# Mikata-Project/adcraft

Hardware: AMD Instinct MI355X
Metric: env-steps/sec (envs×keywords auctions/s) (higher is better)
Workload: dtype i32 cents + f32 (Philox4x32-7 u32); 1 GPU; cfg2: 4096 envs x 256 keywords per GPU, IMPLICIT keywords, mean_volume 128, cvr 0.8, no_vol_prob 0.0, drift False, budget non-binding, 60-step episodes with auto-reset; envs_per_gpu=4096, keywords=256, parallelism=env-sharded x1, collective=none (single GPU), weak_scaling_reference=also.cfg4.value of the N=1 --full line (same per-GPU shard as the N>1 runs)

## Files before the change

adcraft_amd/_ffi.py:

```python
import ctypes as C
import os

from . import build as _build

ADC_OK, ADC_EINVAL, ADC_EHIP, ADC_ENOMEM, ADC_ESTATE, ADC_ETYPE, ADC_ERCCL = 0, -1, -2, -3, -4, -5, -6
MODEL_IMPLICIT, MODEL_EXPLICIT, MODEL_IMPLICIT_GENERAL = 0, 1, 2
P_VOL_MEAN, P_VOL_STD, P_A, P_B, P_BCTR, P_SCTR, P_REV_MEAN, P_REV_STD, P_COUNT = range(9)
(BUF_PARAMS, BUF_BIDS, BUF_BUDGET, BUF_IMPRESSIONS, BUF_CLICKS, BUF_CONVERSIONS, BUF_COST, BUF_REVENUE, BUF_REWARD,
 BUF_CUM_PROFIT, BUF_DAYS, BUF_TERMINATED, BUF_TRUNCATED, BUF_METRIC_PROFIT, BUF_METRIC_SCALARS, BUF_FLAT_OBS,
 BUF_ROLLOUT_ACTION, BUF_ROLLOUT_LOGP, BUF_ROLLOUT_VALUE, BUF_ROLLOUT_REWARD, BUF_ROLLOUT_TERMINATED, BUF_ROLLOUT_TRUNCATED,
 BUF_ROLLOUT_OBS) = range(23)
MLP_TANH, MLP_RELU = 0, 1
ES_CENTERED_RANK, ES_RAW = 0, 1
ES_ADAM, ES_SGD = 0, 1
ROLLOUT_OBS = 1


class EngineError(RuntimeError):
    pass


class EngineStateError(AssertionError):
    """ADC_ESTATE: the call is not valid in the engine's current state (step before reset, a step whose clicks can no longer be
    replayed ...).  An AssertionError, as the reference raises for step-before-reset (gymnasium_kw_env.py:194-196), but one of its
# ... 128 lines not shown
        "adc_engine_stream": ([vp, C.POINTER(vp)], C.c_int),
        "adc_engine_sample_actions": ([vp, f32, f32, f32], C.c_int),
        "adc_engine_set_flat_actions_device": ([vp, vp], C.c_int),
        "adc_engine_flat_obs_enable": ([vp, C.c_int], C.c_int),
        "adc_engine_profile_enable": ([vp, C.c_int], C.c_int),
        "adc_engine_profile_sample_every": ([vp, C.c_int32], C.c_int),
        "adc_engine_profile_read": ([vp, vp, C.POINTER(i64)], C.c_int),
        "adc_engine_profile_records": ([vp, C.POINTER(i64)], C.c_int),
        "adc_engine_region_begin": ([vp], C.c_int),
        "adc_engine_region_end": ([vp, C.POINTER(f64)], C.c_int),
        "adc_engine_comm_stats": ([vp, C.POINTER(i64), C.POINTER(f64), C.POINTER(f64), C.c_int], C.c_int),
        "adc_engine_step_kernel_name": ([vp], C.c_char_p),
        "adc_engine_metrics_enable": ([vp, C.c_int], C.c_int),
        "adc_engine_metrics_reset": ([vp], C.c_int),
        "adc_engine_metrics_read": ([vp, vp, vp], C.c_int),
        "adc_engine_ideal_profit": ([vp, C.c_int, vp, C.c_int, vp], C.c_int),
        "adc_bid_curves_from_samples": ([C.c_int, vp, i32, vp, i32, vp, vp], C.c_int),
        "adc_engine_metrics_akncp_ncp": ([vp, f64, vp, vp], C.c_int),
        "adc_engine_bid_curves_contenders": ([vp, vp, vp, C.POINTER(i32)], C.c_int),
        "adc_engine_outcomes_replay": ([vp, i32, i32, vp, f32, i64, vp, vp, vp, vp, C.POINTER(i64), vp], C.c_int),
        "adc_engine_outcomes_replay_tape": ([vp, i32, vp, f32, C.POINTER(Tape), i64, vp, vp, vp, vp, C.POINTER(i64), vp], C.c_int),
        "adc_nth_price_auction": ([C.c_int, f64, vp, i32, i32, i32, i32, C.POINTER(i32), vp, vp], C.c_int),
        "adc_sigmoid": ([f64, f64, f64], f64),
        "adc_clamp": ([f64, f64, f64], f64),
        "adc_threshold_sigmoid": ([f64, f64, f64, f64], f64),
        "adc_sum_f64": ([vp, i64], f64),
        "adc_count_true": ([vp, i64], i64),
        "adc_nonneg_int_normal": ([f64, f64, u64, u64], u64),
        "adc_binomial": ([u64, f64, u64, u64], u64),
        "adc_cost_create": ([f64, i64, u64, u64, vp], C.c_int),
        "adc_auction_word_intervals": ([f32, f32, f32, f32, vp], C.c_int),
        "adc_auction_word_brackets": ([f32, f32, f32, f32, vp], C.c_int),
        "adc_check_win_brackets": ([i64, vp, vp, vp, vp, vp, vp, vp], i64),
        "adc_sample_random_keyword": ([C.c_uint64, C.c_uint32, C.c_uint32, vp], C.c_int),
        "adc_interp_act_host": ([f32, i32, f32, i32, C.c_double, C.c_double, C.c_double, vp, i32, i32, vp, vp, i32, vp, vp,
                                 C.c_double, vp, vp, vp, vp, vp], C.c_int),
        "adc_interp_key_host": ([f32], C.c_double),
        "adc_engine_mlp_init": ([vp, C.POINTER(MLPConfig), vp], C.c_int),
        "adc_engine_mlp_set_layer": ([vp, i32, i32, vp, vp], C.c_int),
        "adc_engine_mlp_set_norm": ([vp, vp, vp], C.c_int),
        "adc_engine_mlp_set_log_std": ([vp, vp], C.c_int),
        "adc_engine_mlp_set_deterministic": ([vp, i32], C.c_int),
        "adc_engine_mlp_act": ([vp, f32, vp], C.c_int),
        "adc_engine_mlp_step": ([vp, f32], C.c_int),
        "adc_engine_mlp_last": ([vp, vp, vp, vp, vp, vp], C.c_int),
        "adc_engine_mlp_bootstrap_value": ([vp, vp], C.c_int),
        "adc_engine_rollout_enable": ([vp, i32, i32], C.c_int),
        "adc_engine_rollout_reset": ([vp], C.c_int),
        "adc_engine_rollout_fetch": ([vp, C.POINTER(i32), vp, vp, vp, vp, vp, vp, vp], C.c_int),
        "adc_engine_mlp_population": ([vp, i32, vp], C.c_int),
        "adc_engine_mlp_set_member_layer": ([vp, i32, i32, vp, vp], C.c_int),
        "adc_engine_mlp_param_count": ([vp, C.POINTER(i64)], C.c_int),
        "adc_engine_mlp_get_params": ([vp, vp], C.c_int),
        "adc_engine_mlp_get_member_params": ([vp, i32, vp], C.c_int),
        "adc_engine_es_init": ([vp, C.POINTER(ESConfig)], C.c_int),
        "adc_engine_es_perturb": ([vp], C.c_int),
        "adc_engine_es_fitness": ([vp, vp], C.c_int),
        "adc_engine_es_update": ([vp, vp, C.POINTER(ESStats)], C.c_int),
        "adc_engine_es_state_get": ([vp, vp, vp, vp, C.POINTER(i64)], C.c_int),
        "adc_engine_es_state_set": ([vp, vp, vp, vp, i64], C.c_int),
        "adc_es_config_check": ([C.POINTER(ESConfig), C.POINTER(C.c_char_p)], C.c_int),
        "adc_es_noise_host": ([u64, C.c_uint32, C.c_uint32, i64, i64, vp], C.c_int),
        "adc_es_update_host": ([C.POINTER(ESConfig), u64, i32, i64, vp, i64, vp, vp, vp, vp], C.c_int),
        "adc_mlp_config_check": ([C.POINTER(MLPConfig), i32, C.POINTER(C.c_char_p)], C.c_int),
        "adc_mlp_act_host": ([C.POINTER(MLPConfig), i32, vp, vp, vp, vp, vp, vp, vp, vp, vp, u64, C.c_uint32, f32,
                              vp, vp, vp, vp, vp, vp, vp], C.c_int),
        "adc_mlp_math_host": ([i32, f32], f32),
        "adc_mlp_math_sweep_host": ([i32, f32, f32, vp, vp], i64),
        "adc_mlp_agent_key_host": ([u64], u64),
        "adc_mlp_default_agent_key_host": ([u64, u64], u64),
        "adc_explicit_curve_host": ([C.c_uint64, C.c_uint32, i32, i32, f32, f32, f32, vp, i32, vp, vp, vp], C.c_int),
        "adc_debug_win_brackets_device": ([C.c_int, i64, vp, vp, vp, vp, vp], C.c_int),
        "adc_debug_philox_device": ([C.c_int, i64, vp, vp, vp], C.c_int),
        "adc_debug_walk_stats": ([vp, vp, C.c_int], C.c_int),
        "adc_debug_direct_days": ([vp, vp, C.c_int], C.c_int),
        "adc_debug_chain_device": ([C.c_int, f64, i64, vp, vp], C.c_int),
        "adc_engine_env_groups": ([vp, vp], C.c_int),
        "adc_engine_set_env_groups": ([vp, C.c_int32], C.c_int),
        "adc_comm_get_unique_id": ([vp], C.c_int),
        "adc_engine_comm_init": ([vp, vp, i32, i32], C.c_int),
        "adc_engine_comm_destroy": ([vp], C.c_int),
        "adc_engine_comm_info": ([vp, vp, vp], C.c_int),
        "adc_engine_metrics_allreduce": ([vp, vp, vp, vp], C.c_int),
        "adc_engine_comm_allreduce_f64": ([vp, vp, i32, i32], C.c_int),
    }
    for name, (args, res) in sig.items():
        fn = getattr(L, name)
        fn.argtypes = args
        fn.restype = res
    if L.adc_abi_version() != ABI_VERSION or L.adc_stream_revision() != STREAM_REVISION:
        raise EngineError(f"{path}: ABI version {L.adc_abi_version()} / stream revision {L.adc_stream_revision()}, this package "
                          f"expects {ABI_VERSION} / {STREAM_REVISION} (a stale build?)")
    _lib = L
    return L


EXPORTED = None


def check(rc):
    if rc == ADC_OK:
        return
    msg = (lib().adc_last_error() or b"").decode("utf-8", "replace")
    if rc == ADC_EINVAL:
        raise ValueError(msg)
# ... 18 lines not shown
```

adcraft_amd/csrc/adc_law.h:

```cpp
#pragma once
#include <stdint.h>

#if defined(__HIPCC__)
#include <hip/hip_runtime.h>
#define ADC_HD __host__ __device__ __forceinline__
#else
#include <math.h>
#define ADC_HD static inline
#endif

namespace adc {

enum Stage : uint32_t { ST_VOL = 0, ST_AUCTION = 1, ST_DRIFT = 2, ST_XPHANTOM = 3, ST_XREV = 4, ST_ACTION = 5, ST_METRIC = 6, ST_CONV = 7, ST_KEYGEN = 8, ST_AGENT = 9,
                        ST_GBIDDERS = 10, ST_GBID = 11, ST_GCLICK = 12, ST_INTERP = 13, ST_MLP = 14 };
constexpr int kTimesteps = 24;
constexpr int kVolumeMax = 1 << 20;
constexpr float kMoneyMaxCents = 1.0e9f;

struct U4 { uint32_t x, y, z, w; };

ADC_HD uint32_t xor3(uint32_t a, uint32_t b, uint32_t c)
{
#if defined(__HIP_DEVICE_COMPILE__)
    return __builtin_amdgcn_bitop3_b32(a, b, c, 0x96);
// ... 331 lines not shown
ADC_HD int32_t competitor_cents_from_v(uint32_t v24, float loc, float scale, Tab tab)
{
    const float x = fma32(__builtin_fabsf(scale), laplace_deviate_from_v(v24, tab), loc);
    float c = __builtin_rintf(__builtin_fabsf(x) * 100.0f);
    c = c < kMoneyMaxCents ? c : kMoneyMaxCents;
    return (int32_t)c;
}

ADC_HD uint32_t auction_uniform24(uint32_t w, const AuctionLaw &a, bool &click)
{
    click = bernoulli32(w, a.t32);
    const uint32_t d = click ? w : w - a.t32;
    const uint32_t v = mulhi32(d, click ? a.m_click : a.m_noclick);
    return v < 0x00FFFFFFu ? v : 0x00FFFFFFu;
}

ADC_HD bool auction_wins(uint32_t w, int32_t bid_c, int32_t comp_c) { return bid_c > comp_c && w != 0xFFFFFFFFu; }

template <typename Tab>
ADC_HD int32_t auction_outcome_unless_top_word(uint32_t w, const AuctionLaw &a, float loc, float scale, Tab tab, bool &click)
{
    click = w < a.t32;
    const uint32_t d = click ? w : w - a.t32;
    const uint32_t v = mulhi32(d, click ? a.m_click : a.m_noclick);
    return competitor_cents_from_v(v < 0x00FFFFFFu ? v : 0x00FFFFFFu, loc, scale, tab);
}

ADC_HD int32_t auction_outcome(uint32_t w, const AuctionLaw &a, float loc, float scale, const LogTableEntry *tab, bool &click)
{
    return competitor_cents_from_v(auction_uniform24(w, a, click), loc, scale, tab);
}


ADC_HD uint32_t lower_bound_v(int32_t target, float loc, float scale, const LogTableEntry *tab)
{
    const float s = __builtin_fabsf(scale);
    const float x_t = ((float)target - 0.5f) * 0.01f;
    const float z_t = (x_t - loc) / s;
    const float e_t = __builtin_fabsf(z_t);
#if defined(__HIP_DEVICE_COMPILE__)
    float mag_f = __builtin_amdgcn_exp2f(fma32(e_t, -1.44269504f, 23.0f));
#else
    float mag_f = exp2f(fma32(e_t, -1.44269504f, 23.0f));
#endif
    mag_f = mag_f < 8388607.0f ? mag_f : 8388607.0f;
    mag_f = mag_f > 0.0f ? mag_f : 0.0f;
    const uint32_t mag = (uint32_t)mag_f;
    const uint32_t est = z_t < 0.0f ? mag : 0x00FFFFFFu - mag;
    float slack = mag_f * (6.0e-6f + 2.4e-7f * (__builtin_fabsf(x_t) + __builtin_fabsf(loc)) / s);
    slack = slack < 4194304.0f ? slack : 4194304.0f;
    const uint32_t half = 8u + (uint32_t)slack;
    uint32_t lo = est > half ? est - half : 0u;
    uint32_t hi = est + half < 0x01000000u ? est + half : 0x01000000u;
    if (lo > 0u && !(signed_cents_from_v(lo - 1u, loc, scale, tab) < target)) lo = 0u;
    if (hi < 0x01000000u && !(signed_cents_from_v(hi, loc, scale, tab) >= target)) hi = 0x01000000u;
    while (lo < hi) {
        const uint32_t mid = (lo + hi) >> 1;
        if (signed_cents_from_v(mid, loc, scale, tab) >= target) hi = mid;
        else lo = mid + 1u;
    }
    return lo;
}

ADC_HD uint64_t offset_reaching(uint32_t W, uint32_t m, uint64_t range)
{
    if (W == 0u) return 0ull;
    if (W > 0x00FFFFFFu || m == 0u) return range;
    const double q = ((double)W * 4294967296.0) / (double)m;
    if (!(q < (double)range)) return range;
    uint64_t d = (uint64_t)q;
    const uint64_t need = (uint64_t)W << 32;
    if (d * m >= need) { if (d > 0ull && (d - 1ull) * m >= need) d -= 1ull; }
    else { d += 1ull; if (d * m < need) d += 1ull; }
    return d < range ? d : range;
}

struct WinIntervals { uint32_t c_lo, c_w, n_lo, n_w; };

ADC_HD WinIntervals win_intervals(int32_t bid_c, float loc, float scale, uint64_t t_click, const AuctionLaw &law, const LogTableEntry *tab)
{
    const uint32_t w_lo = lower_bound_v(1 - bid_c, loc, scale, tab);
    const uint32_t w_hi = lower_bound_v(bid_c, loc, scale, tab);
    WinIntervals r{0u, 0u, 0u, 0u};
    if (!(w_lo < w_hi)) return r;
    const uint64_t top = 0xFFFFFFFFull;
    uint64_t a = offset_reaching(w_lo, law.m_click, t_click), b = offset_reaching(w_hi, law.m_click, t_click);
    b = b < top ? b : top;
    if (a < b) { r.c_lo = (uint32_t)a; r.c_w = (uint32_t)(b - a); }
    const uint64_t range_n = 4294967296ull - t_click;
    a = t_click + offset_reaching(w_lo, law.m_noclick, range_n);
    b = t_click + offset_reaching(w_hi, law.m_noclick, range_n);
    b = b < top ? b : top;
    if (a < b) { r.n_lo = (uint32_t)a; r.n_w = (uint32_t)(b - a); }
    return r;
}

struct WinBrackets { WinIntervals out, in; };
constexpr float kWordSlack = 4096.0f;

ADC_HD float fast_exp2(float x)
{
#if defined(__HIP_DEVICE_COMPILE__)
    return __builtin_amdgcn_exp2f(x);
#else
    return exp2f(x);
#endif
}
ADC_HD float fast_rcp(float x)
{
#if defined(__HIP_DEVICE_COMPILE__)
    return __builtin_amdgcn_rcpf(x);
#else
    return 1.0f / x;
#endif
}
ADC_HD float min_num(float a, float b) { return __builtin_fminf(a, b); }
ADC_HD float max_num(float a, float b) { return __builtin_fmaxf(a, b); }
ADC_HD uint32_t sat_sub(uint32_t a, uint32_t b)
{
#if defined(__clang__)
    return __builtin_elementwise_sub_sat(a, b);
#else
    return a > b ? a - b : 0u;
#endif
}
ADC_HD uint32_t to_word(float x)
{
#if defined(__HIP_DEVICE_COMPILE__)
    return (uint32_t)x;
#else
    return !(x > 0.0f) ? 0u : x >= 4294967296.0f ? 0xFFFFFFFFu : (uint32_t)x;
#endif
}

ADC_HD void lower_bound_estimate(float x_t, float loc, float inv_s, float &est, float &slack)
{
    const float z_t = (x_t - loc) * inv_s;
    const float e_t = __builtin_fabsf(z_t);
    const float mag = min_num(fast_exp2(fma32(e_t, -1.44269504f, 23.0f)), 8388607.0f);
    est = z_t < 0.0f ? mag : 16777215.0f - mag;
    const float rel = fma32(1.0e-6f, fma32(__builtin_fabsf(x_t) + __builtin_fabsf(loc), inv_s, e_t), 2.0e-5f);
    slack = min_num(fma32(mag, rel, 16.0f), 33554432.0f);
}

ADC_HD WinBrackets win_brackets(int32_t bid_c, float loc, float scale, float t_f)
{
    const float inv_s = fast_rcp(__builtin_fabsf(scale));
    const float bc = (float)bid_c;
    float lo, lo_s, hi, hi_s;
    lower_bound_estimate(fma32(bc, -0.01f, 0.005f), loc, inv_s, lo, lo_s);
    lower_bound_estimate(fma32(bc, 0.01f, -0.005f), loc, inv_s, hi, hi_s);
    const float lo_out = lo - lo_s, lo_in = lo + lo_s, hi_out = hi + hi_s, hi_in = hi - hi_s;
    const float a_c = max_num(t_f * 5.9604644775390625e-08f, 1.0f);
    const float a_n = max_num((4294967296.0f - t_f) * 5.9604644775390625e-08f, 1.0f);
    const float t_dn = t_f - kWordSlack, t_up = t_f + kWordSlack;
    WinBrackets r;
    const uint32_t c_lo_out = to_word(fma32(lo_out, a_c, -kWordSlack)), c_hi_out = to_word(min_num(fma32(hi_out, a_c, kWordSlack), t_f));
    const uint32_t c_lo_in = to_word(fma32(lo_in, a_c, kWordSlack)), c_hi_in = to_word(min_num(fma32(hi_in, a_c, -kWordSlack), t_f));
    const uint32_t n_lo_out = to_word(fma32(lo_out, a_n, t_dn)), n_hi_out = to_word(fma32(hi_out, a_n, t_up));
    const uint32_t n_lo_in = to_word(fma32(lo_in, a_n, t_up)), n_hi_in = to_word(fma32(hi_in, a_n, t_dn));
    r.out = WinIntervals{c_lo_out, sat_sub(c_hi_out, c_lo_out), n_lo_out, sat_sub(n_hi_out, n_lo_out)};
    r.in = WinIntervals{c_lo_in, sat_sub(c_hi_in, c_lo_in), n_lo_in, sat_sub(n_hi_in, n_lo_in)};
    return r;
}

ADC_HD void clicked_win_interval(int32_t bid_c, float loc, float scale, uint64_t t_click, const AuctionLaw &law, const LogTableEntry *tab,
                                 uint32_t &lo, uint32_t &width)
{
    lo = 0u;
    width = 0u;
    const uint32_t w_lo = lower_bound_v(1 - bid_c, loc, scale, tab), w_hi = lower_bound_v(bid_c, loc, scale, tab);
    if (!(w_lo < w_hi)) return;
    const uint64_t a = offset_reaching(w_lo, law.m_click, t_click);
    uint64_t b = offset_reaching(w_hi, law.m_click, t_click);
    b = b < 0xFFFFFFFFull ? b : 0xFFFFFFFFull;
    if (a < b) { lo = (uint32_t)a; width = (uint32_t)(b - a); }
}

ADC_HD int32_t revenue_cents_tab(uint32_t w, float mu, float sd, const NormTableEntry *tab)
{
    float x = fma32(sd, normal_tab(w, tab), mu);
    x = x > 0.01f ? x : 0.01f;
    return money_to_cents(x);
}

ADC_HD int32_t revenue_cents(uint32_t w, float mu, float sd)
{
    float x = fma32(sd, normal_from_word(w), mu);
    x = x > 0.01f ? x : 0.01f;
    return money_to_cents(x);
}

ADC_HD int32_t volume_from_word(uint32_t w, float mean, float sd, const NormTableEntry *tab)
{
    float x = fma32(sd, normal_tab(w, tab), mean);
    x = x > 0.0f ? x : 0.0f;
    x = x < (float)kVolumeMax ? x : (float)kVolumeMax;
    const float t = __builtin_truncf(x);
    return (int32_t)t + ((x - t) >= 0.5f ? 1 : 0);
}

ADC_HD int64_t bid_to_cents(float bid)
{
    double c = __builtin_rint((double)bid * 100.0);
    if (!(c >= 1.0)) c = 1.0;
    if (c > 1.0e9) c = 1.0e9;
    return (int64_t)c;
// ... 289 lines not shown
```

adcraft_amd/csrc/adc_shims.cpp:

```cpp
#include <algorithm>
#include <cmath>
#include <cstdint>
#include <thread>
#include <vector>

#include "../../include/adcraft_engine.h"
#include "adc_law.h"
#include "adc_interp.h"
#include "adc_mlp.h"
#include "adc_es.h"

#define ADC_EXPORT extern "C" __attribute__((visibility("default")))

ADC_EXPORT double adc_sigmoid(double x, double s, double t) { return 1.0 / (1.0 + std::exp(-s * (x - t))); }

ADC_EXPORT double adc_clamp(double x, double lo, double hi) { return x < lo ? lo : (x > hi ? hi : x); }

ADC_EXPORT double adc_threshold_sigmoid(double p, double impression_thresh, double impression_bid_intercept,
                                        double impression_slope)
{
    const double halver = 2.0 + 1e-10;
    const double thresh = adc_clamp(halver * impression_thresh, 0.0, 1.0) / halver;
    const double r = adc_sigmoid(p, impression_slope, impression_bid_intercept);
    return adc_clamp((1.0 + 2.0 * thresh) * r - thresh, 0.0, 1.0);
// ... 84 lines not shown
static inline bool interval_inside(uint32_t a_lo, uint32_t a_w, uint32_t b_lo, uint32_t b_w)
{
    if (a_w == 0u) return true;
    return b_w != 0u && a_lo >= b_lo && (uint64_t)a_lo + a_w <= (uint64_t)b_lo + b_w;
}

ADC_EXPORT int64_t adc_check_win_brackets(int64_t n, const float *bid, const float *cost_loc, const float *cost_scale, const float *buyside_ctr,
                                          const uint32_t *brackets8, int64_t *first_bad, double *ambiguous_words)
{
    if (n < 0 || !bid || !cost_loc || !cost_scale || !buyside_ctr) return -1;
    const adc::LogTableEntry *table = host_log_table();
    int64_t bad = 0, first = -1;
    double amb = 0.0;
    for (int64_t i = 0; i < n; ++i) {
        const int32_t bid_c = (int32_t)adc::bid_to_cents(bid[i]);
        const adc::AuctionLaw law = adc::make_auction_law(buyside_ctr[i]);
        const adc::WinIntervals x = adc::win_intervals(bid_c, cost_loc[i], cost_scale[i], adc::bernoulli_threshold(buyside_ctr[i]), law, table);
        adc::WinBrackets b;
        if (brackets8) {
            const uint32_t *p = brackets8 + 8 * i;
            b.out = adc::WinIntervals{p[0], p[1], p[2], p[3]};
            b.in = adc::WinIntervals{p[4], p[5], p[6], p[7]};
        } else {
            b = adc::win_brackets(bid_c, cost_loc[i], cost_scale[i], adc::bernoulli_threshold_f32(buyside_ctr[i]));
        }
        const bool ok = interval_inside(b.in.c_lo, b.in.c_w, x.c_lo, x.c_w) && interval_inside(x.c_lo, x.c_w, b.out.c_lo, b.out.c_w) &&
                        interval_inside(b.in.n_lo, b.in.n_w, x.n_lo, x.n_w) && interval_inside(x.n_lo, x.n_w, b.out.n_lo, b.out.n_w) &&
                        (uint64_t)b.out.c_lo + b.out.c_w <= 0xFFFFFFFFull && (uint64_t)b.out.n_lo + b.out.n_w <= 0xFFFFFFFFull;
        if (!ok) { if (first < 0) first = i; ++bad; }
        amb += ((double)b.out.c_w - (double)b.in.c_w) + ((double)b.out.n_w - (double)b.in.n_w);
    }
    if (first_bad) *first_bad = first;
    if (ambiguous_words) *ambiguous_words = amb;
    return bad;
}

ADC_EXPORT int adc_sample_random_keyword(uint64_t key, uint32_t keyword, uint32_t serial, float *out8)
{
    if (!out8) return ADC_EINVAL;
    adc::generate_explicit_keyword(key, keyword, serial, out8);
    return ADC_OK;
}

ADC_EXPORT int adc_explicit_curve_host(uint64_t key, uint32_t tick, int32_t keyword, int32_t n_samples, float impression_thresh, float a,
                                       float b, const double *bid_grid, int32_t n_bids, double *ir_out, double *cpc_out, double *z_mid2_out)
{
    if (n_samples <= 0 || n_samples > (1 << 20) || keyword < 0 || n_bids < 0 || (n_bids > 0 && (!bid_grid || !ir_out || !cpc_out)))
        return ADC_EINVAL;
    std::vector<float> z((size_t)n_samples);
    for (int32_t i = 0; i < n_samples; i += 4) {
        const adc::U4 w = adc::draw(key, (uint32_t)(i / 4), adc::ST_METRIC, (uint32_t)keyword, tick);
        const uint32_t ws[4] = {w.x, w.y, w.z, w.w};
        for (int j = 0; j < 4 && i + j < n_samples; ++j) z[(size_t)(i + j)] = adc::normal_from_word(ws[j]);
    }
    std::sort(z.begin(), z.end());
    const float z_lo = z[(size_t)((n_samples - 1) / 2)], z_hi = z[(size_t)(n_samples / 2)];
    if (z_mid2_out) { z_mid2_out[0] = z_lo; z_mid2_out[1] = z_hi; }
    for (int32_t i = 0; i < n_bids; ++i) {
        double mu, sigma;
        adc::explicit_cost_law(bid_grid[i], mu, sigma);
        const adc::CurvePoint q = adc::explicit_curve_point(impression_thresh, a, b, z_lo, z_hi, bid_grid[i], mu, sigma);
        ir_out[i] = q.ir;
        cpc_out[i] = q.cpc;
    }
    return ADC_OK;
}
// ... 243 lines not shown
```

adcraft_amd/csrc/parts/host_api.inc:

```
struct adc_engine {
    adc_config cfg;
    View v;
    hipStream_t stream = nullptr;
    float *d_bids = nullptr, *d_budget = nullptr;
    unsigned char *d_out_block = nullptr, *h_out_block = nullptr;
    size_t out_block_bytes = 0, out_off[10] = {0};
    float *h_act_block = nullptr;
    std::vector<void *> allocs;
    bool have_reset = false;
    int last_step = 0;
    int *h_binding = nullptr;
    size_t rest_table_count = 0;
    size_t click_rec_count = 0;
    bool in_capture = false;
    bool h_binding_off = false;
    bool fail_lazy_alloc = false;
    hipStream_t gstream[4] = {nullptr, nullptr, nullptr, nullptr};
    hipEvent_t ev_fork = nullptr, ev_join[4] = {nullptr, nullptr, nullptr, nullptr};
    int *d_counters = nullptr;
    int last_groups = 1;
    bool api_since_step = true;
    bool needs_fork = true;
    bool groups_pending = false;
    bool stream_exposed = false;
// ... 1724 lines not shown
    launch_ideal_profit(v, 0, 1, n_samples, n_bids, d_grid, d_s, (double *)nullptr, d_ir, d_cpc, (uint2 *)nullptr, lim, 1LL);
    if (hipGetLastError() != hipSuccess || hipDeviceSynchronize() != hipSuccess) return done(fail(ADC_EHIP, "k_ideal_profit failed"));
    if (hipMemcpy(impression_rate_out, d_ir, (size_t)n_bids * 8, hipMemcpyDeviceToHost) != hipSuccess ||
        hipMemcpy(cpc_out, d_cpc, (size_t)n_bids * 8, hipMemcpyDeviceToHost) != hipSuccess)
        return done(fail(ADC_EHIP, "download failed"));
    return done(ADC_OK);
}

ADC_EXPORT int adc_debug_win_brackets_device(int device_id, int64_t n, const float *bid, const float *cost_loc, const float *cost_scale,
                                             const float *buyside_ctr, uint32_t *out8)
{
    if (n < 0 || n > (1 << 26)) return fail(ADC_EINVAL, "n out of range");
    if (n == 0) return ADC_OK;
    if (!bid || !cost_loc || !cost_scale || !buyside_ctr || !out8) return fail(ADC_EINVAL, "NULL argument");
    HIP_TRY(hipSetDevice(device_id));
    float *d_in = nullptr;
    uint32_t *d_out = nullptr;
    auto done = [&](int code) {
        if (d_in) (void)hipFree(d_in);
        if (d_out) (void)hipFree(d_out);
        return code;
    };
    const size_t m = (size_t)n;
    if (hipMalloc((void **)&d_in, 4 * m * 4) != hipSuccess || hipMalloc((void **)&d_out, 8 * m * 4) != hipSuccess) return done(fail(ADC_ENOMEM, "hipMalloc failed"));
    const float *src[4] = {bid, cost_loc, cost_scale, buyside_ctr};
    for (int i = 0; i < 4; ++i)
        if (hipMemcpy(d_in + i * m, src[i], m * 4, hipMemcpyHostToDevice) != hipSuccess) return done(fail(ADC_EHIP, "upload failed"));
    hipLaunchKernelGGL(k_debug_win_brackets, dim3((unsigned)((m + 255) / 256)), dim3(256), 0, 0, (int)n, d_in, d_in + m, d_in + 2 * m, d_in + 3 * m, d_out);
    if (hipGetLastError() != hipSuccess || hipDeviceSynchronize() != hipSuccess) return done(fail(ADC_EHIP, "k_debug_win_brackets failed"));
    if (hipMemcpy(out8, d_out, 8 * m * 4, hipMemcpyDeviceToHost) != hipSuccess) return done(fail(ADC_EHIP, "download failed"));
    return done(ADC_OK);
}

ADC_EXPORT int adc_debug_walk_stats(adc_engine *e, int64_t stats[4], int reset)
{
    ENGINE_GUARD(e);
    if (!stats) return fail(ADC_EINVAL, "stats is NULL");
    HIP_TRY(hipStreamSynchronize(e->stream));
    unsigned long long h[4] = {0, 0, 0, 0};
    HIP_TRY(hipMemcpyFromSymbol(h, HIP_SYMBOL(g_walk_stats), sizeof(h)));
    for (int i = 0; i < 4; ++i) stats[i] = (int64_t)h[i];
#ifdef ADC_EXP_TIMING
    {
        unsigned long long ph[20];
        HIP_TRY(hipMemcpyFromSymbol(ph, HIP_SYMBOL(g_walk_phase), 8 * sizeof(ph[0])));
        std::fprintf(stderr, "walk phases:");
        for (int i = 0; i < 8; ++i) std::fprintf(stderr, " %llu", ph[i]);
        std::fprintf(stderr, "\n");
        HIP_TRY(hipMemcpyFromSymbol(ph, HIP_SYMBOL(g_rest_phase), sizeof(ph)));
        std::fprintf(stderr, "rest-of-day phases (10 ns ticks: pass over the auctions | of which laws | marked cells | outputs | envs | cells walked | of which paid / marks | - | "
                             "list of the marks | k_rest_walk: before the walk | chunks resolved | whole env | slowest env | chunk: cells | chain | paid | at-once variant: own cells | chain | commit | envs):");
        for (int i = 0; i < 20; ++i) std::fprintf(stderr, " %llu", ph[i]);
        std::fprintf(stderr, "\n");
        if (reset) {
            const unsigned long long z8[8] = {0, 0, 0, 0, 0, 0, 0, 0};
            HIP_TRY(hipMemcpyToSymbol(HIP_SYMBOL(g_walk_phase), z8, sizeof(z8)));
            const unsigned long long z16[20] = {0, 0, 0, 0, 0, 0, 0, 0, 0, 0, 0, 0, 0, 0, 0, 0, 0, 0, 0, 0};
            HIP_TRY(hipMemcpyToSymbol(HIP_SYMBOL(g_rest_phase), z16, sizeof(z16)));
        }
    }
#endif
    if (reset) {
        const unsigned long long z[4] = {0, 0, 0, 0};
        HIP_TRY(hipMemcpyToSymbol(HIP_SYMBOL(g_walk_stats), z, sizeof(z)));
    }
    return ADC_OK;
// ... 1417 lines not shown
```

adcraft_amd/csrc/parts/kernel_sparse.inc:

```
constexpr int kSparseItemCap = 1024;

struct SparseShared {
    int2 offvol[kFastBlock + 1];
    adc::WinIntervals win_out[kFastBlock], win_in[kFastBlock];
    KwLawA law_a[kFastBlock];
    float2 rev_law[kFastBlock];
    unsigned long long a_cnt[kFastBlock], a_cost[kFastBlock], a_rev[kFastBlock];
    float lognodes[adc::kLogTableIntervals + 1];
    float normtab[adc::kNormTableEntries + 1];
    unsigned char items[kSparseItemCap];
    uint2 queue[kFastBlock / kWave][kQueueCap];
    int wave_tot[kFastBlock / kWave];
};
static_assert(sizeof(SparseShared) <= 25 * 1280, "SparseShared must allow 5 workgroups per CU");
static_assert(kSparseItemCap % kFastBlock == 0, "a round of work items lies on one side of the list's end");

__device__ __forceinline__ unsigned long long wave_sum_u64_limbs(unsigned long long x)
{
    const unsigned int lo = (unsigned int)x, hi = (unsigned int)(x >> 32);
    const unsigned long long a = (unsigned int)wave_sum_i32((int)(lo & 0x3FFFFFu));
    const unsigned long long b = (unsigned int)wave_sum_i32((int)((lo >> 22) | ((hi & 0xFFFu) << 10)));
    const unsigned long long c = (unsigned int)wave_sum_i32((int)(hi >> 12));
    return a + (b << 22) + (c << 44);
}
// ... 337 lines not shown
            const long long s = (long long)metric_old + (rv - my_cost);
            if (s == (long long)(int)s) lane_elem(a->metric_lo + o, tid) = (int)s;
            else { lane_elem(a->metric_hi + o, tid) += s; lane_elem(a->metric_lo + o, tid) = 0; }
        }
    }
    if (!more || (tile_index + 1) / tiles != env) {
        const unsigned long long c = wave_sum_u64_limbs(acc_cost), p = wave_sum_u64_limbs(acc_rev);
        if (lane == 0u && (c | p) != 0ull) {
            ArgView *a = args();
            atomicAdd((unsigned long long *)&a->env_cost[env], c);
            atomicAdd((unsigned long long *)&a->env_profit[env], p - c);
        }
        acc_cost = acc_rev = 0ull;
    }
    FDBG_ADD(5, FDBG_T() - t_p3);
    FDBG_ADD(6, 1);
  }
#ifdef ADC_EXP_TIMING
    fdbg[1] = FDBG_T() - t_kernel;
    if (tid == 0u) for (int i = 0; i < 8; ++i) atomicAdd(&g_fdbg[blockIdx.x & 255][i], fdbg[i]);
#endif
}

__global__ void k_debug_win_brackets(int n, const float *bid, const float *loc, const float *scale, const float *bctr, uint32_t *out8)
{
    const int i = blockIdx.x * blockDim.x + threadIdx.x;
    if (i >= n) return;
    const adc::WinBrackets b = adc::win_brackets(adc::bid_to_cents_i32(bid[i]), loc[i], scale[i], adc::bernoulli_threshold_f32(bctr[i]));
    uint32_t *o = out8 + 8 * (size_t)i;
    o[0] = b.out.c_lo; o[1] = b.out.c_w; o[2] = b.out.n_lo; o[3] = b.out.n_w;
    o[4] = b.in.c_lo; o[5] = b.in.c_w; o[6] = b.in.n_lo; o[7] = b.in.n_w;
}

__global__ void k_debug_philox(int n, const uint32_t *ctr4, const uint32_t *key2, uint32_t *out4)
{
    const int i = blockIdx.x * blockDim.x + threadIdx.x;
    if (i >= n) return;
    const adc::U4 w = adc::philox4x32(ctr4[4 * i], ctr4[4 * i + 1], ctr4[4 * i + 2], ctr4[4 * i + 3], key2[2 * i], key2[2 * i + 1]);
    out4[4 * i] = w.x; out4[4 * i + 1] = w.y; out4[4 * i + 2] = w.z; out4[4 * i + 3] = w.w;
}
```

include/adcraft_engine.h:

```cpp
#ifndef ADCRAFT_ENGINE_H
#define ADCRAFT_ENGINE_H

#include <stddef.h>
#include <stdint.h>

#ifdef __cplusplus
extern "C" {
#endif

#define ADC_ABI_VERSION 5
#define ADC_STREAM_REVISION 5

typedef enum adc_status {
    ADC_OK = 0,
    ADC_EINVAL = -1,
    ADC_EHIP = -2,
    ADC_ENOMEM = -3,
    ADC_ESTATE = -4,
    ADC_ETYPE = -5,
    ADC_ERCCL = -6
} adc_status;

typedef enum adc_model {
    ADC_MODEL_IMPLICIT = 0,
// ... 255 lines not shown
typedef struct adc_es_stats {
    int64_t generation;
    double fitness_mean, fitness_max, fitness_min;
    double grad_norm, theta_norm;
} adc_es_stats;
int adc_engine_es_init(adc_engine *e, const adc_es_config *cfg);
int adc_engine_es_perturb(adc_engine *e);
int adc_engine_es_fitness(adc_engine *e, double *fitness_m);
int adc_engine_es_update(adc_engine *e, const double *fitness_m, adc_es_stats *stats);
int adc_engine_es_state_get(adc_engine *e, float *theta_p, float *m_p, float *v_p, int64_t *generation);
int adc_engine_es_state_set(adc_engine *e, const float *theta_p, const float *m_p, const float *v_p, int64_t generation);

int adc_engine_outcomes_replay(adc_engine *e, int32_t env, int32_t steps_back, const float *bids_k, float budget, int64_t capacity,
                               int32_t *keyword, int32_t *timestep, double *cost, double *revenue, int64_t *count, int32_t *share_volume_k);
int adc_engine_outcomes_replay_tape(adc_engine *e, int32_t env, const float *bids_k, float budget, const adc_tape *tape, int64_t capacity,
                                    int32_t *keyword, int32_t *timestep, double *cost, double *revenue, int64_t *count, int32_t *share_volume_k);

int adc_nth_price_auction(int device_id, double bid, const double *other_bids, int32_t n_auctions, int32_t n_bidders,
                          int32_t n, int32_t num_winners, int32_t *impressions, int32_t *placements, double *costs);

double adc_sigmoid(double x, double s, double t);
double adc_clamp(double x, double lo, double hi);
double adc_threshold_sigmoid(double p, double impression_thresh,
                             double impression_bid_intercept, double impression_slope);
double adc_sum_f64(const double *x, int64_t n);
int64_t adc_count_true(const uint8_t *x, int64_t n);
uint64_t adc_nonneg_int_normal(double mean, double std, uint64_t seed, uint64_t counter);
uint64_t adc_binomial(uint64_t n, double p, uint64_t seed, uint64_t counter);
int adc_cost_create(double x, int64_t n, uint64_t seed, uint64_t counter, double *out_n);
int adc_auction_word_intervals(float bid, float cost_loc, float cost_scale, float buyside_ctr, uint32_t *out4);
int adc_auction_word_brackets(float bid, float cost_loc, float cost_scale, float buyside_ctr, uint32_t *out8);
int64_t adc_check_win_brackets(int64_t n, const float *bid, const float *cost_loc, const float *cost_scale, const float *buyside_ctr,
                               const uint32_t *brackets8, int64_t *first_bad, double *ambiguous_words);
int adc_sample_random_keyword(uint64_t key, uint32_t keyword, uint32_t serial, float *out8);
int adc_explicit_curve_host(uint64_t key, uint32_t tick, int32_t keyword, int32_t n_samples, float impression_thresh, float a, float b,
                            const double *bid_grid, int32_t n_bids, double *ir_out, double *cpc_out, double *z_mid2_out);
int adc_interp_act_host(float ave_rpc, int32_t num_rpc_obs, float ave_sctr, int32_t num_sctr_obs, double max_observed,
                        double profit_acquisition_threshold, double bid_step, const double *allowed_bids, int32_t n_bids,
                        int32_t n_clicks, const uint16_t *clicks_cent, const float *ave_clicks, int32_t n_cpc, const uint16_t *cpc_cent,
                        const double *ave_cpc, double u, double *margin_out, double *cost_out, double *bid_out, int32_t *index_out,
                        double *mass_out);
double adc_interp_key_host(float bid);
int adc_mlp_act_host(const adc_mlp_config *cfg, int32_t num_keywords, const float *obs_d, const float *const *policy_w,
                     const float *const *policy_b, const float *const *value_w, const float *const *value_b, const float *shift_d,
                     const float *scale_d, const float *log_std_a, const float *normals_a, uint64_t agent_key, uint32_t tick,
                     float budget_override, float *mean_a, float *log_std_out_a, float *action_a, float *logp, float *value,
                     float *bids_k, float *budget);
int adc_es_config_check(const adc_es_config *cfg, const char **message);
int adc_es_noise_host(uint64_t seed, uint32_t pair, uint32_t generation, int64_t p0, int64_t n, float *eps_n);
int adc_es_update_host(const adc_es_config *cfg, uint64_t seed, int32_t members, int64_t n_params, const double *fitness_m, int64_t generation,
                       float *theta_p, float *m_p, float *v_p, float *grad_p);
int adc_mlp_config_check(const adc_mlp_config *cfg, int32_t num_keywords, const char **message);
float adc_mlp_math_host(int32_t fn, float x);
int64_t adc_mlp_math_sweep_host(int32_t fn, float lo, float hi, double *out3, int64_t *violations4);
uint64_t adc_mlp_agent_key_host(uint64_t seed);
uint64_t adc_mlp_default_agent_key_host(uint64_t engine_seed, uint64_t global_env_id);
int adc_debug_philox_device(int device_id, int64_t n, const uint32_t *ctr4, const uint32_t *key2, uint32_t *out4);
int adc_debug_chain_device(int device_id, double r0, int64_t n, const double *x, double *out2);
int adc_debug_walk_stats(adc_engine *e, int64_t stats[4], int reset);
int adc_debug_direct_days(adc_engine *e, int64_t *env_days, int reset);
int adc_debug_win_brackets_device(int device_id, int64_t n, const float *bid, const float *cost_loc, const float *cost_scale,
                                  const float *buyside_ctr, uint32_t *out8);

#ifdef __cplusplus
}
#endif
#endif
```

Baseline: 6.442 billion keyword-steps/s.

## Replace win-interval binary searches with seeded narrow probes and reciprocal-based offset solve

The full 24-bit binary search that finds the win-word bounds is replaced. The new code seeds an estimate from an inverse-CDF approximation and bisects only a small window around it, using cached log-table cells. When the window check fails it falls back to the wide search. offset_reaching swaps an iterative or division-based solve for a double-precision reciprocal multiply plus a ±1 correction. Host and device checkers are added to compare against the kept reference versions; the added exactness logic risks divergence and more branching.

```diff
diff --git a/adcraft_amd/_ffi.py b/adcraft_amd/_ffi.py
--- a/adcraft_amd/_ffi.py
+++ b/adcraft_amd/_ffi.py
@@ -184,6 +184,8 @@
         "adc_auction_word_intervals": ([f32, f32, f32, f32, vp], C.c_int),
         "adc_auction_word_brackets": ([f32, f32, f32, f32, vp], C.c_int),
         "adc_check_win_brackets": ([i64, vp, vp, vp, vp, vp, vp, vp], i64),
+        "adc_check_win_intervals": ([i64, vp, vp, vp, vp, vp, vp, vp], i64),
+        "adc_check_offset_reaching": ([i64, vp, vp, vp, vp], i64),
         "adc_sample_random_keyword": ([C.c_uint64, C.c_uint32, C.c_uint32, vp], C.c_int),
         "adc_interp_act_host": ([f32, i32, f32, i32, C.c_double, C.c_double, C.c_double, vp, i32, i32, vp, vp, i32, vp, vp,
                                  C.c_double, vp, vp, vp, vp, vp], C.c_int),
@@ -223,6 +225,7 @@
         "adc_mlp_default_agent_key_host": ([u64, u64], u64),
         "adc_explicit_curve_host": ([C.c_uint64, C.c_uint32, i32, i32, f32, f32, f32, vp, i32, vp, vp, vp], C.c_int),
         "adc_debug_win_brackets_device": ([C.c_int, i64, vp, vp, vp, vp, vp], C.c_int),
+        "adc_debug_win_intervals_device": ([C.c_int, i64, vp, vp, vp, vp, vp, vp], C.c_int),
         "adc_debug_philox_device": ([C.c_int, i64, vp, vp, vp], C.c_int),
         "adc_debug_walk_stats": ([vp, vp, C.c_int], C.c_int),
         "adc_debug_direct_days": ([vp, vp, C.c_int], C.c_int),
diff --git a/adcraft_amd/csrc/adc_law.h b/adcraft_amd/csrc/adc_law.h
--- a/adcraft_amd/csrc/adc_law.h
+++ b/adcraft_amd/csrc/adc_law.h
@@ -387,7 +387,7 @@
 }
 
 
-ADC_HD uint32_t lower_bound_v(int32_t target, float loc, float scale, const LogTableEntry *tab)
+ADC_HD uint32_t lower_bound_v_ref(int32_t target, float loc, float scale, const LogTableEntry *tab)
 {
     const float s = __builtin_fabsf(scale);
     const float x_t = ((float)target - 0.5f) * 0.01f;
@@ -417,7 +417,7 @@
     return lo;
 }
 
-ADC_HD uint64_t offset_reaching(uint32_t W, uint32_t m, uint64_t range)
+ADC_HD uint64_t offset_reaching_ref(uint32_t W, uint32_t m, uint64_t range)
 {
     if (W == 0u) return 0ull;
     if (W > 0x00FFFFFFu || m == 0u) return range;
@@ -432,26 +432,23 @@
 
 struct WinIntervals { uint32_t c_lo, c_w, n_lo, n_w; };
 
-ADC_HD WinIntervals win_intervals(int32_t bid_c, float loc, float scale, uint64_t t_click, const AuctionLaw &law, const LogTableEntry *tab)
-{
-    const uint32_t w_lo = lower_bound_v(1 - bid_c, loc, scale, tab);
-    const uint32_t w_hi = lower_bound_v(bid_c, loc, scale, tab);
+ADC_HD WinIntervals win_intervals_ref(int32_t bid_c, float loc, float scale, uint64_t t_click, const AuctionLaw &law, const LogTableEntry *tab)
+{
+    const uint32_t w_lo = lower_bound_v_ref(1 - bid_c, loc, scale, tab);
+    const uint32_t w_hi = lower_bound_v_ref(bid_c, loc, scale, tab);
     WinIntervals r{0u, 0u, 0u, 0u};
     if (!(w_lo < w_hi)) return r;
     const uint64_t top = 0xFFFFFFFFull;
-    uint64_t a = offset_reaching(w_lo, law.m_click, t_click), b = offset_reaching(w_hi, law.m_click, t_click);
+    uint64_t a = offset_reaching_ref(w_lo, law.m_click, t_click), b = offset_reaching_ref(w_hi, law.m_click, t_click);
     b = b < top ? b : top;
     if (a < b) { r.c_lo = (uint32_t)a; r.c_w = (uint32_t)(b - a); }
     const uint64_t range_n = 4294967296ull - t_click;
-    a = t_click + offset_reaching(w_lo, law.m_noclick, range_n);
-    b = t_click + offset_reaching(w_hi, law.m_noclick, range_n);
+    a = t_click + offset_reaching_ref(w_lo, law.m_noclick, range_n);
+    b = t_click + offset_reaching_ref(w_hi, law.m_noclick, range_n);
     b = b < top ? b : top;
     if (a < b) { r.n_lo = (uint32_t)a; r.n_w = (uint32_t)(b - a); }
     return r;
 }
-
-struct WinBrackets { WinIntervals out, in; };
-constexpr float kWordSlack = 4096.0f;
 
 ADC_HD float fast_exp2(float x)
 {
@@ -469,6 +466,170 @@
     return 1.0f / x;
 #endif
 }
+
+struct ProbeCell {
+    uint32_t key;
+    float a, c0, base, slope, value, ef, ss;
+};
+
+template <typename Tab>
+ADC_HD ProbeCell probe_cell(float v, float s_abs, Tab tab)
+{
+    const uint32_t v24 = (uint32_t)v;
+    const uint32_t neg_mask = 0u - (v24 >> 23);
+    const uint32_t mag = (v24 ^ neg_mask) & 0x007FFFFFu;
+    const uint32_t bits = float_to_bits(fma32((float)mag, 2.0f, 1.0f));
+    const LogTableEntry t = log_entry(tab, (bits & 0x007FFFFFu) >> 15);
+    const bool pos = neg_mask != 0u;
+    const float base = bits_to_float(bits & 0xFFFF8000u);
+    ProbeCell c;
+    c.ef = (float)((int)(bits >> 23) - 151);
+    c.value = t.value;
+    c.slope = t.slope * bits_to_float((277u - (bits >> 23)) << 23);
+    c.a = pos ? -2.0f : 2.0f;
+    c.c0 = pos ? 33554430.0f : 1.0f;
+    c.base = pos ? base - 1.0f : base;
+    c.ss = pos ? -s_abs : s_abs;
+    c.key = float_to_bits(fma32(v, c.a, c.c0)) >> 15;
+    return c;
+}
+
+template <typename Tab>
+ADC_HD float probe_x(ProbeCell &c, float v, float loc, float s_abs, Tab tab)
+{
+    float w = fma32(v, c.a, c.c0);
+    if ((float_to_bits(w) >> 15) != c.key) {
+        c = probe_cell(v, s_abs, tab);
+        w = fma32(v, c.a, c.c0);
+    }
+    float r = fma32(c.slope, w - c.base, c.value);
+    r = fma32(c.ef, -2.12194440e-4f, r);
+    r = fma32(c.ef, 0.693359375f, r);
+    return fma32(c.ss, r, loc);
+}
+ADC_HD bool cents_reach(float x, float tf) { return !(__builtin_rintf(x * 100.0f) < tf); }
+
+template <typename Tab>
+ADC_HD uint32_t lower_bound_v_wide(int32_t target, float loc, float scale, Tab tab)
+{
+    uint32_t lo = 0u, hi = 0x01000000u;
+    while (lo < hi) {
+        const uint32_t mid = (lo + hi) >> 1;
+        if (signed_cents_from_v(mid, loc, scale, tab) >= target) hi = mid;
+        else lo = mid + 1u;
+    }
+    return lo;
+}
+
+constexpr float kWinWindowMax = 2048.0f;
+constexpr float kWinRounding = 1.2e-7f;
+
+template <typename Tab>
+ADC_HD int win_bounds_v(int32_t bid_c, float loc, float scale, Tab tab, uint32_t &w_lo, uint32_t &w_hi)
+{
+    const float s = __builtin_fabsf(scale);
+    const float inv_s = fast_rcp(s);
+    const float tf[2] = {(float)(1 - bid_c), (float)bid_c};
+    ProbeCell cell[2];
+    float pos[2], first[2], step[2], last[2];
+    int wide[2];
+#pragma unroll
+    for (int b = 0; b < 2; ++b) {
+        const float x_t = (tf[b] - 0.5f) * 0.01f;
+        const float z_t = (x_t - loc) * inv_s;
+        float mag = fast_exp2(fma32(__builtin_fabsf(z_t), -1.44269504f, 23.0f));
+        mag = mag < 8388607.0f ? mag : 8388607.0f;
+        mag = mag > 0.0f ? mag : 0.0f;
+        const float fl = __builtin_floorf(mag);
+        const float est = z_t < 0.0f ? fl : 16777215.0f - fl;
+        cell[b] = probe_cell(est, s, tab);
+        const float x0 = probe_x(cell[b], est, loc, s, tab);
+        float dv = __builtin_rintf((x_t - x0) * mag * inv_s);
+        dv = dv < 16777216.0f ? dv : 0.0f;
+        dv = dv > -16777216.0f ? dv : 0.0f;
+        float e2 = est + dv;
+        e2 = e2 > 0.0f ? e2 : 0.0f;
+        e2 = e2 < 16777215.0f ? e2 : 16777215.0f;
+        float h = fma32(mag * inv_s, kWinRounding * (__builtin_fabsf(x_t) + __builtin_fabsf(loc)), 3.0f);
+        h = h < 1.0e9f ? h : 1.0e9f;
+        wide[b] = (int)!(h <= kWinWindowMax && bid_c <= 8388608);
+        const float half = bits_to_float((float_to_bits(h) + 0x007FFFFFu) & 0x7F800000u);
+        const float top = (16777216.0f - (half + half)) + 1.0f;
+        float f = e2 - half;
+        f = f > 0.0f ? f : 0.0f;
+        f = f < top ? f : top;
+        first[b] = pos[b] = f;
+        step[b] = wide[b] ? 0.0f : half;
+        last[b] = f + ((half + half) - 1.0f);
+        const bool reach0 = cents_reach(x0, tf[b]);
+        if (est == 0.0f && reach0) { first[b] = pos[b] = 0.0f; step[b] = 0.0f; last[b] = -1.0f; }
+        if (est == 16777215.0f && !reach0) { first[b] = 0.0f; pos[b] = 16777216.0f; step[b] = 0.0f; last[b] = -1.0f; }
+    }
+    while (step[0] >= 1.0f || step[1] >= 1.0f) {
+#pragma unroll
+        for (int b = 0; b < 2; ++b) {
+            if (step[b] >= 1.0f) {
+                const float x = probe_x(cell[b], pos[b] + (step[b] - 1.0f), loc, s, tab);
+                pos[b] = cents_reach(x, tf[b]) ? pos[b] : pos[b] + step[b];
+                step[b] *= 0.5f;
+            }
+        }
+    }
+#pragma unroll
+    for (int b = 0; b < 2; ++b) {
+        const bool at_first = pos[b] == first[b] && first[b] > 0.0f;
+        const bool at_last = pos[b] == last[b] && pos[b] < 16777216.0f;
+        if (!wide[b] && (at_first | at_last)) {
+            const bool reach = cents_reach(probe_x(cell[b], at_first ? first[b] - 1.0f : pos[b], loc, s, tab), tf[b]);
+            wide[b] = (int)(reach == at_first);
+        }
+    }
+    w_lo = wide[0] ? lower_bound_v_wide(1 - bid_c, loc, scale, tab) : (uint32_t)pos[0];
+    w_hi = wide[1] ? lower_bound_v_wide(bid_c, loc, scale, tab) : (uint32_t)pos[1];
+    return wide[0] + wide[1];
+}
+
+ADC_HD uint64_t offset_reaching(uint32_t W, uint32_t m, double inv_m, uint64_t range)
+{
+    const double q = ((double)W * 4294967296.0) * inv_m;
+    const double qc = q < 4294967295.0 ? q : 4294967295.0;
+    const uint64_t d = (uint64_t)(uint32_t)qc;
+    const uint64_t need = (uint64_t)W << 32, mm = (uint64_t)m;
+    const uint64_t p = d * mm;
+    const uint64_t down = (d > 0ull && p - mm >= need) ? d - 1ull : d;
+    const uint64_t up = p + mm >= need ? d + 1ull : d + 2ull;
+    uint64_t r = p >= need ? down : up;
+    r = r < range ? r : range;
+    const bool none = W > 0x00FFFFFFu || m == 0u || !(q < (double)range);
+    return W == 0u ? 0ull : none ? range : r;
+}
+
+template <typename Tab>
+ADC_HD WinIntervals win_intervals(int32_t bid_c, float loc, float scale, uint64_t t_click, const AuctionLaw &law, Tab tab, int *wide_paths = nullptr)
+{
+    uint32_t w_lo, w_hi;
+    const int wide = win_bounds_v(bid_c, loc, scale, tab, w_lo, w_hi);
+    if (wide_paths) *wide_paths = wide;
+    WinIntervals r{0u, 0u, 0u, 0u};
+    if (!(w_lo < w_hi)) return r;
+    const double inv_c = 1.0 / (double)(law.m_click != 0u ? law.m_click : 1u);
+    const double inv_n = 1.0 / (double)(law.m_noclick != 0u ? law.m_noclick : 1u);
+    const uint64_t top = 0xFFFFFFFFull;
+    const uint64_t range_n = 4294967296ull - t_click;
+    const uint64_t ca = offset_reaching(w_lo, law.m_click, inv_c, t_click);
+    uint64_t cb = offset_reaching(w_hi, law.m_click, inv_c, t_click);
+    const uint64_t na = t_click + offset_reaching(w_lo, law.m_noclick, inv_n, range_n);
+    uint64_t nb = t_click + offset_reaching(w_hi, law.m_noclick, inv_n, range_n);
+    cb = cb < top ? cb : top;
+    nb = nb < top ? nb : top;
+    if (ca < cb) { r.c_lo = (uint32_t)ca; r.c_w = (uint32_t)(cb - ca); }
+    if (na < nb) { r.n_lo = (uint32_t)na; r.n_w = (uint32_t)(nb - na); }
+    return r;
+}
+
+struct WinBrackets { WinIntervals out, in; };
+constexpr float kWordSlack = 4096.0f;
+
 ADC_HD float min_num(float a, float b) { return __builtin_fminf(a, b); }
 ADC_HD float max_num(float a, float b) { return __builtin_fmaxf(a, b); }
 ADC_HD uint32_t sat_sub(uint32_t a, uint32_t b)
@@ -524,10 +685,12 @@
 {
     lo = 0u;
     width = 0u;
-    const uint32_t w_lo = lower_bound_v(1 - bid_c, loc, scale, tab), w_hi = lower_bound_v(bid_c, loc, scale, tab);
+    uint32_t w_lo, w_hi;
+    win_bounds_v(bid_c, loc, scale, tab, w_lo, w_hi);
     if (!(w_lo < w_hi)) return;
-    const uint64_t a = offset_reaching(w_lo, law.m_click, t_click);
-    uint64_t b = offset_reaching(w_hi, law.m_click, t_click);
+    const double inv_m = 1.0 / (double)(law.m_click != 0u ? law.m_click : 1u);
+    const uint64_t a = offset_reaching(w_lo, law.m_click, inv_m, t_click);
+    uint64_t b = offset_reaching(w_hi, law.m_click, inv_m, t_click);
     b = b < 0xFFFFFFFFull ? b : 0xFFFFFFFFull;
     if (a < b) { lo = (uint32_t)a; width = (uint32_t)(b - a); }
 }
diff --git a/adcraft_amd/csrc/adc_shims.cpp b/adcraft_amd/csrc/adc_shims.cpp
--- a/adcraft_amd/csrc/adc_shims.cpp
+++ b/adcraft_amd/csrc/adc_shims.cpp
@@ -140,6 +140,43 @@
     }
     if (first_bad) *first_bad = first;
     if (ambiguous_words) *ambiguous_words = amb;
+    return bad;
+}
+
+ADC_EXPORT int64_t adc_check_win_intervals(int64_t n, const float *bid, const float *cost_loc, const float *cost_scale, const float *buyside_ctr,
+                                           const uint32_t *intervals4, int64_t *first_bad, int64_t *wide_keywords)
+{
+    if (n < 0 || !bid || !cost_loc || !cost_scale || !buyside_ctr) return -1;
+    const adc::LogTableEntry *table = host_log_table();
+    int64_t bad = 0, first = -1, wide = 0;
+    for (int64_t i = 0; i < n; ++i) {
+        const int32_t bid_c = (int32_t)adc::bid_to_cents(bid[i]);
+        const adc::AuctionLaw law = adc::make_auction_law(buyside_ctr[i]);
+        const uint64_t t_click = adc::bernoulli_threshold(buyside_ctr[i]);
+        const adc::WinIntervals x = adc::win_intervals_ref(bid_c, cost_loc[i], cost_scale[i], t_click, law, table);
+        int w = 0;
+        adc::WinIntervals y = adc::win_intervals(bid_c, cost_loc[i], cost_scale[i], t_click, law, table, &w);
+        wide += w != 0;
+        if (intervals4) {
+            const uint32_t *p = intervals4 + 4 * i;
+            y = adc::WinIntervals{p[0], p[1], p[2], p[3]};
+        }
+        if (x.c_lo != y.c_lo || x.c_w != y.c_w || x.n_lo != y.n_lo || x.n_w != y.n_w) { if (first < 0) first = i; ++bad; }
+    }
+    if (first_bad) *first_bad = first;
+    if (wide_keywords) *wide_keywords = wide;
+    return bad;
+}
+
+ADC_EXPORT int64_t adc_check_offset_reaching(int64_t n, const uint32_t *W, const uint32_t *m, const uint64_t *range, int64_t *first_bad)
+{
+    if (n < 0 || !W || !m || !range) return -1;
+    int64_t bad = 0, first = -1;
+    for (int64_t i = 0; i < n; ++i) {
+        const double inv_m = 1.0 / (double)(m[i] != 0u ? m[i] : 1u);
+        if (adc::offset_reaching(W[i], m[i], inv_m, range[i]) != adc::offset_reaching_ref(W[i], m[i], range[i])) { if (first < 0) first = i; ++bad; }
+    }
+    if (first_bad) *first_bad = first;
     return bad;
 }
 
diff --git a/adcraft_amd/csrc/parts/host_api.inc b/adcraft_amd/csrc/parts/host_api.inc
--- a/adcraft_amd/csrc/parts/host_api.inc
+++ b/adcraft_amd/csrc/parts/host_api.inc
@@ -1780,6 +1780,38 @@
     return done(ADC_OK);
 }
 
+ADC_EXPORT int adc_debug_win_intervals_device(int device_id, int64_t n, const float *bid, const float *cost_loc, const float *cost_scale,
+                                              const float *buyside_ctr, uint32_t *out4, int64_t *wide_keywords)
+{
+    if (n < 0 || n > (1 << 26)) return fail(ADC_EINVAL, "n out of range");
+    if (wide_keywords) *wide_keywords = 0;
+    if (n == 0) return ADC_OK;
+    if (!bid || !cost_loc || !cost_scale || !buyside_ctr || !out4) return fail(ADC_EINVAL, "NULL argument");
+    HIP_TRY(hipSetDevice(device_id));
+    float *d_in = nullptr;
+    uint32_t *d_out = nullptr;
+    auto done = [&](int code) {
+        if (d_in) (void)hipFree(d_in);
+        if (d_out) (void)hipFree(d_out);
+        return code;
+    };
+    const size_t m = (size_t)n;
+    if (hipMalloc((void **)&d_in, 4 * m * 4) != hipSuccess || hipMalloc((void **)&d_out, 4 * m * 4 + 8) != hipSuccess) return done(fail(ADC_ENOMEM, "hipMalloc failed"));
+    unsigned long long *d_wide = (unsigned long long *)(d_out + 4 * m);
+    if (hipMemset(d_wide, 0, 8) != hipSuccess) return done(fail(ADC_EHIP, "hipMemset failed"));
+    const float *src[4] = {bid, cost_loc, cost_scale, buyside_ctr};
+    for (int i = 0; i < 4; ++i)
+        if (hipMemcpy(d_in + i * m, src[i], m * 4, hipMemcpyHostToDevice) != hipSuccess) return done(fail(ADC_EHIP, "upload failed"));
+    hipLaunchKernelGGL(k_build_log_table, dim3((adc::kNormTableEntries + 256) / 256), dim3(256), 0, 0);
+    hipLaunchKernelGGL(k_debug_win_intervals, dim3((unsigned)((m + 255) / 256)), dim3(256), 0, 0, (int)n, d_in, d_in + m, d_in + 2 * m, d_in + 3 * m, d_out, d_wide);
+    if (hipGetLastError() != hipSuccess || hipDeviceSynchronize() != hipSuccess) return done(fail(ADC_EHIP, "k_debug_win_intervals failed"));
+    unsigned long long h_wide = 0;
+    if (hipMemcpy(out4, d_out, 4 * m * 4, hipMemcpyDeviceToHost) != hipSuccess || hipMemcpy(&h_wide, d_wide, 8, hipMemcpyDeviceToHost) != hipSuccess)
+        return done(fail(ADC_EHIP, "download failed"));
+    if (wide_keywords) *wide_keywords = (int64_t)h_wide;
+    return done(ADC_OK);
+}
+
 ADC_EXPORT int adc_debug_walk_stats(adc_engine *e, int64_t stats[4], int reset)
 {
     ENGINE_GUARD(e);
diff --git a/adcraft_amd/csrc/parts/kernel_sparse.inc b/adcraft_amd/csrc/parts/kernel_sparse.inc
--- a/adcraft_amd/csrc/parts/kernel_sparse.inc
+++ b/adcraft_amd/csrc/parts/kernel_sparse.inc
@@ -393,6 +393,19 @@
     o[4] = b.in.c_lo; o[5] = b.in.c_w; o[6] = b.in.n_lo; o[7] = b.in.n_w;
 }
 
+__global__ void k_debug_win_intervals(int n, const float *bid, const float *loc, const float *scale, const float *bctr, uint32_t *out4,
+                                      unsigned long long *wide)
+{
+    const int i = blockIdx.x * blockDim.x + threadIdx.x;
+    if (i >= n) return;
+    int w = 0;
+    const adc::WinIntervals r = adc::win_intervals(adc::bid_to_cents_i32(bid[i]), loc[i], scale[i], adc::bernoulli_threshold(bctr[i]),
+                                                   adc::make_auction_law(bctr[i]), g_log_table, &w);
+    uint32_t *o = out4 + 4 * (size_t)i;
+    o[0] = r.c_lo; o[1] = r.c_w; o[2] = r.n_lo; o[3] = r.n_w;
+    if (w != 0) atomicAdd(wide, 1ull);
+}
+
 __global__ void k_debug_philox(int n, const uint32_t *ctr4, const uint32_t *key2, uint32_t *out4)
 {
     const int i = blockIdx.x * blockDim.x + threadIdx.x;
diff --git a/include/adcraft_engine.h b/include/adcraft_engine.h
--- a/include/adcraft_engine.h
+++ b/include/adcraft_engine.h
@@ -311,6 +311,9 @@
 int adc_auction_word_brackets(float bid, float cost_loc, float cost_scale, float buyside_ctr, uint32_t *out8);
 int64_t adc_check_win_brackets(int64_t n, const float *bid, const float *cost_loc, const float *cost_scale, const float *buyside_ctr,
                                const uint32_t *brackets8, int64_t *first_bad, double *ambiguous_words);
+int64_t adc_check_win_intervals(int64_t n, const float *bid, const float *cost_loc, const float *cost_scale, const float *buyside_ctr,
+                                const uint32_t *intervals4, int64_t *first_bad, int64_t *wide_keywords);
+int64_t adc_check_offset_reaching(int64_t n, const uint32_t *W, const uint32_t *m, const uint64_t *range, int64_t *first_bad);
 int adc_sample_random_keyword(uint64_t key, uint32_t keyword, uint32_t serial, float *out8);
 int adc_explicit_curve_host(uint64_t key, uint32_t tick, int32_t keyword, int32_t n_samples, float impression_thresh, float a, float b,
                             const double *bid_grid, int32_t n_bids, double *ir_out, double *cpc_out, double *z_mid2_out);
@@ -340,6 +343,8 @@
 int adc_debug_direct_days(adc_engine *e, int64_t *env_days, int reset);
 int adc_debug_win_brackets_device(int device_id, int64_t n, const float *bid, const float *cost_loc, const float *cost_scale,
                                   const float *buyside_ctr, uint32_t *out8);
+int adc_debug_win_intervals_device(int device_id, int64_t n, const float *bid, const float *cost_loc, const float *cost_scale,
+                                   const float *buyside_ctr, uint32_t *out4, int64_t *wide_keywords);
 
 #ifdef __cplusplus
 }
```

Result: no change. 6.499 billion keyword-steps/s, median of 6 (+0.9%).
